# thucz/splatter360

Hardware: AMD Instinct MI355X
Metric: Msplats/s fwd+bwd @1M Gaussians, 1024x512 ERP (higher is better)
Workload: dtype f32; 1 GPU; BASELINE configs[2]: 1048576 encoder-like synthetic Gaussians (seed 0, deg-4 SH, from 2 context panoramas 1024x512), 1024x512 ERP = 6 faces 256x256 + stitch, fwdbwd, L2 loss on faces (fused epilogue, scalar reduced in the backward's first launch), lean tile lists; gaussians=1048576, face=256, views_per_gpu=1, parallelism=view-sharded x1, num_rendered=2237238, visible_pairs=1096454, split_lists=auto, split_quadrants=0, wide_rectangles=0, workspace_bytes_forward=1086440448, workspace_bytes_backward=1062934272, max_instances=2862083

## Files before the change

splatter360_amd/csrc/s360_forward.hip:

```cpp
#include "s360_device.h"
#include "s360_prof.h"
#include "s360_adapter_math.h"

#include <cstdio>
#include <cstdlib>

namespace s360 {

typedef float f4v __attribute__((ext_vector_type(4)));

template <bool CH_MAJOR, bool JAC>
__global__ __launch_bounds__(S360_BLOCK) void k_sh_eval(KParams kp, const S360View* __restrict__ views,
                                                       const float* __restrict__ means, const float* __restrict__ shs,
                                                       float4* __restrict__ rgbc, float* __restrict__ sh_jac,
                                                       uint32_t* __restrict__ zero_ptr, int zero_words) {
    const int g = blockIdx.x * S360_BLOCK + threadIdx.x;
    if (g < zero_words) zero_ptr[g] = 0u;
    if (g >= kp.P) return;
    const bool fast = kp.M == 25 && kp.deg == 4;
    const float* sh = shs + (size_t)g * kp.M * 3;
    float c[75];
    if (fast) load75(sh, c);
    const S360View& vw = views[0];
    const float sc = vw.scale;
// ... 682 lines not shown
        const uint32_t nch1 = nc1 > SORT_SHORT ? (nc1 + SORT_CHUNK - 1) / SORT_CHUNK : 0u;
        if (nch0 || nch1) atomicAdd(&lds_nlong, (nch0 ? 1u : 0u) + (nch1 ? 1u : 0u));
        uint32_t ctot;
        const uint32_t cex0 = block_exclusive_scan<TS_BLOCK / 64>(nch0 + nch1, lds, ctot), cex1 = cex0 + nch0;
        if (i0 < nt) {
            tile_start[i0] = carry + ex0;
            tile_cursor[i0] = 0;
            tile_max_contrib[i0] = 0;
            chunk_start[i0] = ccarry + cex0;
        }
        if (i1 < nt) {
            tile_start[i1] = carry + ex1;
            tile_cursor[i1] = 0;
            tile_max_contrib[i1] = 0;
            chunk_start[i1] = ccarry + cex1;
        }
        carry += tot;
        ccarry += ctot;
    }
    atomicMax(&lds_max, mx);
    __syncthreads();
    if (threadIdx.x == 0) {
        chunk_start[nt] = ccarry;
        tile_start[nt] = carry;
        header[0] = carry;
        header[1] = carry > cap ? 1u : 0u;
        header[2] = lds_max;
        {
            const uint32_t nmax = min(lds_max, cap);
            const uint32_t nch = nmax > SORT_SHORT ? (nmax + SORT_CHUNK - 1) / SORT_CHUNK : 0u;
            header[3] = merge_passes_of(nch);
        }
        header[4] = 0;
        *reinterpret_cast<SegBufs*>(header + S360_HDR_SEGBUFS) = sg_in;
        header[S360_HDR_SPLIT] = 0;
        header[6] = header[7] = 0;
        header[S360_HDR_SORT_ERR_TILE] = header[S360_HDR_SORT_ERR_PASS] = 0;
        if (header_mirror) __hip_atomic_store(header_mirror, (unsigned long long)carry | ((unsigned long long)(carry > cap ? 1u : 0u) << 32) |
                                                             ((unsigned long long)ccarry << 33),
                                              __ATOMIC_RELAXED, __HIP_MEMORY_SCOPE_SYSTEM);
        header[S360_HDR_NLONG] = lds_nlong;
        for (int i = 8; i < 25; ++i) header[i] = 0;
    }
}

#ifndef S360_EMIT_PPT
#define S360_EMIT_PPT 4
#endif
constexpr int EMIT_PPT = S360_EMIT_PPT;

template <bool LDS_BIN, bool COOP = false>
__global__ __launch_bounds__(S360_BLOCK) void k_emit(KParams kp, const uint32_t* __restrict__ tiles_touched,
                                                    const uint8_t* __restrict__ vis_mask, const float4* __restrict__ recA, const float4* __restrict__ recC,
                                                    const float* __restrict__ depths, const uint32_t* __restrict__ tile_start,
                                                    uint32_t* __restrict__ tile_cursor, uint64_t* __restrict__ keys,
                                                    uint2* __restrict__ slot_info, uint32_t* __restrict__ slot_pair,
                                                    uint32_t* __restrict__ slot_ticket, uint32_t* __restrict__ header,
                                                    uint32_t* __restrict__ long_pairs) {
    extern __shared__ __attribute__((aligned(16))) uint32_t lds_bin[];
    __shared__ uint32_t s_scan[S360_BLOCK / 64];
    __shared__ uint32_t s_slot0;
    const int v = blockIdx.y;
    const int g0 = blockIdx.x * (S360_BLOCK * EMIT_PPT) + threadIdx.x;
    const size_t tb = (size_t)image_of_view(kp, v) * kp.T;
    uint32_t* cnt = lds_bin;
    uint32_t* base = lds_bin + kp.T;
    const bool lean = (kp.flags & S360_FLAG_LEAN_LISTS) != 0;
    if (LDS_BIN) {
        for (int i = threadIdx.x; i < kp.T; i += S360_BLOCK) cnt[i] = 0u;
        __syncthreads();
    }
    __shared__ uint32_t s_p[S360_BLOCK * EMIT_PPT];
    uint32_t vis = 0;
#pragma unroll
    for (int j = 0; j < EMIT_PPT; ++j) {
        const int g = g0 + j * S360_BLOCK;
        if (g < kp.P && ((vis_mask[g] >> v) & 1u)) vis |= 1u << j;
    }
    uint32_t nvis;
    {
        uint32_t off = block_exclusive_scan((uint32_t)__builtin_popcount(vis), s_scan, nvis);
        for (uint32_t m = vis; m; m &= m - 1) s_p[off++] = (uint32_t)v * (uint32_t)kp.P + (uint32_t)(g0 + __builtin_ctz(m) * S360_BLOCK);
    }
    __syncthreads();
    uint32_t pr[EMIT_PPT], tt[EMIT_PPT], rlo[EMIT_PPT], rhi[EMIT_PPT], dbits[EMIT_PPT], hm[EMIT_PPT];
#pragma unroll
    for (int j = 0; j < EMIT_PPT; ++j) {
        const uint32_t e = threadIdx.x + j * S360_BLOCK;
        tt[j] = 0u; pr[j] = 0u; rlo[j] = rhi[j] = dbits[j] = 0u; hm[j] = 0xFFFFFFFFu;
        if (e < nvis) {
            const uint32_t p = s_p[e];
            const float4 rc = recA[3 * (size_t)p + 2];
            const float4 ra = recA[3 * (size_t)p];
            pr[j] = p;
            tt[j] = tiles_touched[p];
            dbits[j] = __float_as_uint(depths[p]);
            int minx, miny, maxx, maxy;
            tile_rect(ra.x, ra.y, __float_as_int(rc.y), kp.gx, kp.gy, minx, miny, maxx, maxy);
            rlo[j] = (uint32_t)minx | ((uint32_t)miny << 16);
            rhi[j] = (uint32_t)maxx | ((uint32_t)maxy << 16);
            if (lean && (maxx - minx) * (maxy - miny) <= 32) hm[j] = slot_info[p].y;
        }
    }
    uint32_t sl[EMIT_PPT], ticket = 0;
#pragma unroll
    for (int j = 0; j < EMIT_PPT; ++j) sl[j] = 0u;
    if (slot_pair) {
        uint32_t carry = 0;
#pragma unroll
        for (int j = 0; j < EMIT_PPT; ++j) {
            if ((uint32_t)j * S360_BLOCK >= nvis) break;
            uint32_t tot;
            sl[j] = carry + block_exclusive_scan(tt[j], s_scan, tot);
            carry += tot;
        }
        if (threadIdx.x == 0 && carry) ticket = tile_start[tb] + atomicAdd(&slot_ticket[image_of_view(kp, v) * 64], carry);
    }
    const int lane = threadIdx.x & 63;
    if (LDS_BIN) {
#pragma unroll
        for (int j = 0; j < EMIT_PPT; ++j) {
            if (COOP && (uint32_t)j * S360_BLOCK >= nvis) break;
            const bool wide = COOP && tt[j] > 32u;
            if (tt[j] && !wide) {
                const int minx = rlo[j] & 0xFFFFu, miny = rlo[j] >> 16, maxx = rhi[j] & 0xFFFFu, maxy = rhi[j] >> 16;
                uint32_t m = hm[j];
                for (int y = miny; y < maxy; ++y)
                    for (int x = minx; x < maxx; ++x) {
                        if (m & 1u) atomicAdd(&cnt[y * kp.gx + x], 1u);
                        m = (m >> 1) | 0x80000000u;
                    }
            }
            if (COOP) {
                for (unsigned long long big = __ballot(wide); big; big &= big - 1ull) {
                    const int src = (int)__builtin_ctzll(big);
                    const uint32_t lo = (uint32_t)__shfl((int)rlo[j], src), hi = (uint32_t)__shfl((int)rhi[j], src);
                    const int minx = lo & 0xFFFFu, miny = lo >> 16, w = (int)(hi & 0xFFFFu) - minx, n = w * ((int)(hi >> 16) - miny);
                    for (int i = lane; i < n; i += 64) {
                        const int y = i / w;
                        atomicAdd(&cnt[(miny + y) * kp.gx + minx + (i - y * w)], 1u);
                    }
                }
            }
        }
        __syncthreads();
        for (int i = threadIdx.x; i < kp.T; i += S360_BLOCK) {
            const uint32_t c = cnt[i];
            if (c) {
                base[i] = tile_start[tb + i] + atomicAdd(&tile_cursor[tb + i], c);
                cnt[i] = 0u;
            }
        }
    }
    if (slot_pair || LDS_BIN) {
        if (slot_pair && threadIdx.x == 0) s_slot0 = ticket;
        __syncthreads();
    }
#pragma unroll
    for (int j = 0; j < EMIT_PPT; ++j) {
        if (COOP && (uint32_t)j * S360_BLOCK >= nvis) break;
        const bool wide = COOP && tt[j] > 32u;
        const uint32_t p = pr[j];
        uint32_t slot = 0;
        if (tt[j]) {
            if (slot_pair) {
                slot = sl[j] + s_slot0;
                slot_info[p].x = slot;
            }
            if (tt[j] > 32u) {
                const uint32_t k = atomicAdd(&header[4], 1u);
                if (slot_pair && k < kp.cap / 32u + 1u) long_pairs[k] = p;
            }
        }
        const uint32_t ptag = p | (tt[j] > 32u ? 0x80000000u : 0u);
        if (tt[j] && !wide) {
            const int minx = rlo[j] & 0xFFFFu, miny = rlo[j] >> 16, maxx = rhi[j] & 0xFFFFu, maxy = rhi[j] >> 16;
            const uint64_t key = ((uint64_t)dbits[j] << 32) | (uint64_t)p;
            uint32_t m = hm[j];
            for (int y = miny; y < maxy; ++y)
                for (int x = minx; x < maxx; ++x) {
                    if (m & 1u) {
                        const int t = y * kp.gx + x;
                        const uint32_t pos = LDS_BIN ? base[t] + atomicAdd(&cnt[t], 1u)
                                                     : tile_start[tb + t] + atomicAdd(&tile_cursor[tb + t], 1u);
                        if (pos < kp.cap) keys[pos] = key;
                        if (slot_pair) {
                            if (slot < kp.cap) slot_pair[slot] = ptag;
                            ++slot;
                        }
                    }
                    m = (m >> 1) | 0x80000000u;
                }
        }
        if (COOP) {
            for (unsigned long long big = __ballot(wide); big; big &= big - 1ull) {
                const int src = (int)__builtin_ctzll(big);
                const uint32_t lo = (uint32_t)__shfl((int)rlo[j], src), hi = (uint32_t)__shfl((int)rhi[j], src);
                const uint32_t ps = (uint32_t)__shfl((int)p, src), ds = (uint32_t)__shfl((int)dbits[j], src), s0 = (uint32_t)__shfl((int)slot, src);
                const uint64_t key = ((uint64_t)ds << 32) | (uint64_t)ps;
                const int minx = lo & 0xFFFFu, miny = lo >> 16, w = (int)(hi & 0xFFFFu) - minx, n = w * ((int)(hi >> 16) - miny);
                for (int i = lane; i < n; i += 64) {
                    const int y = i / w;
                    const int t = (miny + y) * kp.gx + minx + (i - y * w);
                    const uint32_t pos = LDS_BIN ? base[t] + atomicAdd(&cnt[t], 1u)
                                                 : tile_start[tb + t] + atomicAdd(&tile_cursor[tb + t], 1u);
                    if (pos < kp.cap) keys[pos] = key;
                    if (slot_pair && s0 + (uint32_t)i < kp.cap) slot_pair[s0 + (uint32_t)i] = ps | 0x80000000u;
                }
            }
        }
    }
}

__device__ __forceinline__ uint64_t ld_dev(const uint64_t* p) { return __hip_atomic_load(p, __ATOMIC_RELAXED, __HIP_MEMORY_SCOPE_AGENT); }
__device__ __forceinline__ void st_dev(uint64_t* p, uint64_t v) { __hip_atomic_store(p, v, __ATOMIC_RELAXED, __HIP_MEMORY_SCOPE_AGENT); }

template <int THREADS, int E, bool DEV = false>
__device__ __forceinline__ void block_merge_sort(const uint64_t* __restrict__ in, uint64_t* __restrict__ out,
                                                 uint32_t* __restrict__ list, uint32_t n, uint64_t* lds_m) {
#define S360_PHYS(i) ((i) + (i) / E)
    const int tid = threadIdx.x;
    uint64_t k[E];
#pragma unroll
    for (int q = 0; q < E; ++q) {
        const uint32_t i = (uint32_t)(tid * E + q);
        k[q] = i < n ? in[i] : ~0ull;
    }
#pragma unroll
    for (int r = 0; r < E; ++r) {
#pragma unroll
        for (int q = (r & 1); q + 1 < E; q += 2) {
            const uint64_t a = k[q], b = k[q + 1];
            k[q] = a < b ? a : b;
            k[q + 1] = a < b ? b : a;
        }
    }
#pragma unroll
    for (int q = 0; q < E; ++q) lds_m[S360_PHYS((uint32_t)(tid * E + q))] = k[q];
#define S360_SORT_SYNC(w)                                                      \
    do {                                                                       \
        if (2u * (w) <= 64u * E) {                                             \
            __builtin_amdgcn_fence(__ATOMIC_RELEASE, "wavefront");             \
            __builtin_amdgcn_wave_barrier();                                   \
            __builtin_amdgcn_fence(__ATOMIC_ACQUIRE, "wavefront");             \
        } else {                                                               \
            __syncthreads();                                                   \
        }                                                                      \
    } while (0)
    S360_SORT_SYNC(E);
    uint32_t npad = E;
    while (npad < n) npad <<= 1;
    const uint32_t out0 = (uint32_t)tid * E;
    const bool live = out0 < n;
    for (uint32_t width = E; width < npad; width <<= 1) {
        const uint32_t pair = out0 / (2 * width) * (2 * width);
        const uint32_t pa = pair, pb = pair + width;
#define S360_A(x) lds_m[S360_PHYS(pa + (x))]
#define S360_B(x) lds_m[S360_PHYS(pb + (x))]
        if (live) {
            const uint32_t diag = out0 - pair;
            uint32_t lo_a = diag > width ? diag - width : 0u, hi_a = diag < width ? diag : width;
            while (lo_a < hi_a) {
                const uint32_t mid = (lo_a + hi_a) >> 1;
                if (S360_A(mid) <= S360_B(diag - 1 - mid)) lo_a = mid + 1; else hi_a = mid;
            }
            uint32_t a = lo_a, b = diag - lo_a;
            uint64_t ka = a < width ? S360_A(a) : ~0ull, kb = b < width ? S360_B(b) : ~0ull;
#pragma unroll
            for (int q = 0; q < E; ++q) {
                const bool take_a = ka <= kb;
                k[q] = take_a ? ka : kb;
                if (take_a) {
                    ++a;
                    ka = a < width ? S360_A(a) : ~0ull;
                } else {
                    ++b;
                    kb = b < width ? S360_B(b) : ~0ull;
                }
            }
        }
        S360_SORT_SYNC(width);
        if (live) {
#pragma unroll
            for (int q = 0; q < E; ++q) lds_m[S360_PHYS(out0 + q)] = k[q];
        }
        S360_SORT_SYNC(2u * width);
#undef S360_A
#undef S360_B
    }
    __syncthreads();
#undef S360_SORT_SYNC
#pragma unroll
    for (int q = 0; q < E; ++q) {
        const uint32_t i = (uint32_t)(tid * E + q);
        if (i < n) {
            const uint64_t kq = lds_m[S360_PHYS(i)];
            if (DEV) st_dev(out + i, kq); else out[i] = kq;
            if (list) list[i] = (uint32_t)kq;
        }
    }
#undef S360_PHYS
}


struct ChunkUnit {
    uint32_t s, n, k, passes, t;
    bool valid;
};
__device__ __forceinline__ ChunkUnit chunk_unit(const uint32_t* __restrict__ tile_start, const uint32_t* __restrict__ chunk_start,
                                                 int nt, uint32_t cap, uint32_t b) {
    ChunkUnit u;
    u.valid = b < chunk_start[nt];
    u.s = u.n = u.k = u.passes = u.t = 0;
    if (!u.valid) return u;
    const int lane = threadIdx.x & 63;
    int lo = 0, hi = nt;
    while (hi - lo > 1) {
        const int step = (hi - lo + 63) / 64;
        const int t = lo + lane * step;
        const bool p = t < hi && chunk_start[t] <= b;
        const int cnt = __popcll(__ballot(p));
        const int nhi = lo + cnt * step;
        lo = lo + (cnt - 1) * step;
        hi = nhi < hi ? nhi : hi;
    }
    u.s = min(tile_start[lo], cap);
    u.n = min(tile_start[lo + 1], cap) - u.s;
    u.k = b - chunk_start[lo];
    u.t = (uint32_t)lo;
    u.passes = merge_passes_of((u.n + SORT_CHUNK - 1) / SORT_CHUNK);
    return u;
}

__device__ __forceinline__ uint32_t merge_path_global_wave(const uint64_t* __restrict__ A, uint32_t la,
                                                           const uint64_t* __restrict__ B, uint32_t lb, uint32_t d, int lane) {
    uint32_t lo = d > lb ? d - lb : 0u, hi = d < la ? d : la;
    while (lo < hi) {
        const uint32_t step = (hi - lo + 63u) / 64u;
        const uint32_t a = lo + (uint32_t)lane * step;
        const bool p = a < hi && ld_dev(A + a) <= ld_dev(B + (d - 1 - a));
        const uint32_t cnt = (uint32_t)__popcll(__ballot(p));
        if (cnt == 0) {
            hi = lo;
        } else {
            const uint32_t nhi = lo + cnt * step;
            lo = lo + (cnt - 1) * step + 1;
            hi = nhi < hi ? nhi : hi;
        }
    }
    return lo;
}

__device__ __forceinline__ void merge_unit(const ChunkUnit& u, uint32_t pass, uint64_t* __restrict__ keys,
                                           uint64_t* __restrict__ alt, uint32_t* __restrict__ list, uint64_t* lds_m, uint32_t* s_part) {
    constexpr int THREADS = SORT_THREADS, E = 8;
#define S360_PHYS(i) ((i) + (i) / E)
    const uint32_t R = SORT_CHUNK << pass;
    const uint32_t o_tile = u.k * SORT_CHUNK, len = min(SORT_CHUNK, u.n - o_tile);
    const uint32_t pair0 = o_tile / (2 * R) * (2 * R);
    const uint32_t la = min(R, u.n - pair0), lb = min(R, u.n - pair0 - la);
    const uint64_t* src = (((u.passes - pass) & 1u) ? alt : keys) + u.s + pair0;
    uint64_t* dst = (((u.passes - pass - 1) & 1u) ? alt : keys) + u.s + o_tile;
    const uint64_t* A = src;
    const uint64_t* B = src + la;
    const uint32_t o = o_tile - pair0;
    if (threadIdx.x < 128) {
        const int w = threadIdx.x >> 6;
        const uint32_t r = merge_path_global_wave(A, la, B, lb, o + (uint32_t)w * len, threadIdx.x & 63);
        if ((threadIdx.x & 63) == 0) s_part[w] = r;
    }
    __syncthreads();
    const uint32_t a0 = s_part[0], a1 = s_part[1], b0 = o - a0, b1 = o + len - a1;
    const uint32_t na = a1 - a0, nb = b1 - b0;
    {
        uint64_t kin[E];
#pragma unroll
        for (int q = 0; q < E; ++q) {
            const uint32_t i = (uint32_t)threadIdx.x + (uint32_t)q * THREADS;
            kin[q] = i < len ? ld_dev(i < na ? A + (a0 + i) : B + (b0 + (i - na))) : 0ull;
        }
#pragma unroll
        for (int q = 0; q < E; ++q) {
            const uint32_t i = (uint32_t)threadIdx.x + (uint32_t)q * THREADS;
            if (i < len) lds_m[S360_PHYS(i)] = kin[q];
        }
    }
    __syncthreads();
    const uint32_t out0 = (uint32_t)threadIdx.x * E;
    if (out0 < len) {
        uint32_t lo_a = out0 > nb ? out0 - nb : 0u, hi_a = out0 < na ? out0 : na;
        while (lo_a < hi_a) {
            const uint32_t mid = (lo_a + hi_a) >> 1;
            if (lds_m[S360_PHYS(mid)] <= lds_m[S360_PHYS(na + out0 - 1 - mid)]) lo_a = mid + 1; else hi_a = mid;
        }
        uint32_t a = lo_a, b = out0 - lo_a;
        uint64_t ka = a < na ? lds_m[S360_PHYS(a)] : ~0ull, kb = b < nb ? lds_m[S360_PHYS(na + b)] : ~0ull;
        const bool last_pass = pass + 1 == u.passes;
        uint32_t* lst = list + u.s + o_tile;
#pragma unroll
        for (int q = 0; q < E; ++q) {
            const bool take_a = ka <= kb;
            const uint64_t kq = take_a ? ka : kb;
            if (take_a) {
                ++a;
                ka = a < na ? lds_m[S360_PHYS(a)] : ~0ull;
            } else {
                ++b;
                kb = b < nb ? lds_m[S360_PHYS(na + b)] : ~0ull;
            }
            if (out0 + q < len) {
                st_dev(dst + (out0 + q), kq);
                if (last_pass) lst[out0 + q] = (uint32_t)kq;
            }
        }
    }
#undef S360_PHYS
}

template <int THREADS>
__device__ __forceinline__ void sort_tiles_global_body(const uint32_t* __restrict__ tile_start, uint64_t* __restrict__ keys,
                                                       uint32_t* __restrict__ list, uint32_t lo, uint32_t cap, int nt,
                                                       uint32_t first, uint32_t stride) {
  for (int tile = (int)first; tile < nt; tile += (int)stride) {
    const uint32_t s = min(tile_start[tile], cap), e = min(tile_start[tile + 1], cap);
    const uint32_t n = e - s;
    if (n <= lo) continue;
    uint32_t npad = 1;
    while (npad < n) npad <<= 1;
    uint64_t* kk = keys + s;
    for (uint32_t k = 2; k <= npad; k <<= 1) {
        const uint32_t half = k >> 1;
        for (uint32_t t = threadIdx.x; t < (npad >> 1); t += THREADS) {
            const uint32_t blk = t / half, off = t - blk * half;
            const uint32_t i = blk * k + off, l = blk * k + (k - 1 - off);
            if (l < n) {
                const uint64_t a = kk[i], b = kk[l];
                if (a > b) {
                    kk[i] = b;
                    kk[l] = a;
                }
            }
        }
        __threadfence_block();
        __syncthreads();
        for (uint32_t j = k >> 2; j > 0; j >>= 1) {
            for (uint32_t t = threadIdx.x; t < (npad >> 1); t += THREADS) {
                const uint32_t i = ((t & ~(j - 1)) << 1) | (t & (j - 1)), l = i | j;
                if (l < n) {
                    const uint64_t a = kk[i], b = kk[l];
                    if (a > b) {
                        kk[i] = b;
                        kk[l] = a;
                    }
                }
            }
            __threadfence_block();
            __syncthreads();
        }
    }
    for (uint32_t i = threadIdx.x; i < n; i += THREADS) list[s + i] = (uint32_t)kk[i];
    __syncthreads();
  }
}

#ifndef S360_MERGE_BLOCKS
#define S360_MERGE_BLOCKS 256
#endif
__device__ __forceinline__ bool wait_count(const uint32_t* counter, uint32_t need) {
    uint32_t spins = 0;
    while (__hip_atomic_load(counter, __ATOMIC_RELAXED, __HIP_MEMORY_SCOPE_AGENT) < need) {
        if (++spins > (uint32_t)S360_SEGS_SPINS) return false;
        __builtin_amdgcn_s_sleep(32);
    }
    return true;
}
__device__ __forceinline__ void drain_stores_and_sync() {
    asm volatile("s_waitcnt vmcnt(0)" ::: "memory");
    __builtin_amdgcn_fence(__ATOMIC_RELEASE, "workgroup");
    __syncthreads();
}
__global__ __launch_bounds__(SORT_THREADS) void k_sort_stage1(const uint32_t* __restrict__ tile_start, const uint32_t* __restrict__ chunk_start,
                                                    int nt, uint64_t* __restrict__ keys, uint64_t* __restrict__ alt,
                                                    uint32_t* __restrict__ list, uint32_t cap, uint32_t max_passes, uint32_t cgrid,
                                                    const uint32_t* __restrict__ tile_count, uint32_t* __restrict__ tile_order,
                                                    uint32_t* __restrict__ header, unsigned long long* __restrict__ wide_mirror,
                                                    uint32_t* __restrict__ merge_done, uint32_t mgrid, uint32_t global_lo) {
    extern __shared__ __attribute__((aligned(16))) uint64_t lds_m[];
    uint32_t* const queue = merge_done + (size_t)nt * MAX_PASSES;
    uint32_t* const chunks_sorted = queue + 1;
    const uint32_t bid = blockIdx.x;
    if (bid < cgrid) {
        const uint32_t nchunks = chunk_start[nt];
        for (uint32_t b = bid; b < nchunks; b += cgrid) {
            const ChunkUnit u = chunk_unit(tile_start, chunk_start, nt, cap, b);
            if (u.valid && u.passes <= max_passes) {
                const uint32_t c0 = u.k * SORT_CHUNK, len = min(SORT_CHUNK, u.n - c0);
                uint64_t* dst = ((u.passes & 1u) ? alt : keys) + u.s + c0;
                if (u.passes == 0) {
                    block_merge_sort<SORT_THREADS, 8>(keys + u.s + c0, dst, list + u.s, len, lds_m);
                } else {
                    block_merge_sort<SORT_THREADS, 8, true>(keys + u.s + c0, dst, nullptr, len, lds_m);
                    drain_stores_and_sync();
                    if (threadIdx.x == 0) __hip_atomic_fetch_add(&chunks_sorted[u.t], 1u, __ATOMIC_RELAXED, __HIP_MEMORY_SCOPE_AGENT);
                }
            }
            __syncthreads();
        }
        return;
    }
    if (bid < cgrid + mgrid) {
        __shared__ uint32_t s_part[2];
        __shared__ uint32_t s_ticket;
        const uint32_t npass = min(header[3], max_passes);
        const uint32_t nchunks = npass ? chunk_start[nt] : 0u;
        const uint32_t nunits = npass * nchunks;
        while (bid - cgrid < nunits) {
            if (threadIdx.x == 0) s_ticket = __hip_atomic_fetch_add(queue, 1u, __ATOMIC_RELAXED, __HIP_MEMORY_SCOPE_AGENT);
            __syncthreads();
            const uint32_t tk = s_ticket;
            __syncthreads();
            if (tk >= nunits) break;
            const uint32_t pass = tk / nchunks, blk = tk - pass * nchunks;
            const ChunkUnit u = chunk_unit(tile_start, chunk_start, nt, cap, blk);
            if (!u.valid || u.passes > max_passes || pass >= u.passes) continue;
            const uint32_t nch = (u.n + SORT_CHUNK - 1) / SORT_CHUNK;
            if (threadIdx.x == 0) {
                const bool ok = wait_count(pass ? &merge_done[(size_t)u.t * MAX_PASSES + pass - 1] : &chunks_sorted[u.t], nch);
                if (!ok && atomicAdd(&header[7], 0x1000000u) < 0x1000000u) { header[S360_HDR_SORT_ERR_TILE] = u.t; header[S360_HDR_SORT_ERR_PASS] = pass; }
                s_ticket = ok ? 1u : 0u;
            }
            __syncthreads();
            const bool ok = s_ticket != 0u;
            __syncthreads();
            if (!ok) return;
            merge_unit(u, pass, keys, alt, list, lds_m, s_part);
            drain_stores_and_sync();
            if (threadIdx.x == 0 && pass + 1 < u.passes)
                __hip_atomic_fetch_add(&merge_done[(size_t)u.t * MAX_PASSES + pass], 1u, __ATOMIC_RELAXED, __HIP_MEMORY_SCOPE_AGENT);
        }
        if (header[2] > global_lo) sort_tiles_global_body<SORT_THREADS>(tile_start, keys, list, global_lo, cap, nt, bid - cgrid, mgrid);
        return;
    }
    if (bid < cgrid + mgrid + (uint32_t)nt) {
        const uint32_t tile = bid - cgrid - mgrid;
        const uint32_t s = min(tile_start[tile], cap), e = min(tile_start[tile + 1], cap);
        const uint32_t n = e - s;
        if (n == 0 || n > SORT_SHORT) return;
        block_merge_sort<SORT_THREADS, (int)(SORT_SHORT / SORT_THREADS)>(keys + s, keys + s, list + s, n, lds_m);
        return;
    }
    if (wide_mirror && threadIdx.x == 0) __hip_atomic_store(wide_mirror, (unsigned long long)header[4], __ATOMIC_RELAXED, __HIP_MEMORY_SCOPE_SYSTEM);
    if (tile_order) order_units_body<SORT_THREADS>(tile_count, tile_order, nt);
}

#ifndef S360_SPARSE_PIXELS
#define S360_SPARSE_PIXELS 6
#endif
constexpr int SPARSE_PIXELS = S360_SPARSE_PIXELS;

struct MseEp {
    const float* target;
    float* d_images;
    float* partials;
    float grad_scale;
    float* loss_out;
};

__global__ __launch_bounds__(MSE_BLOCK) void k_mse_finish(const float* __restrict__ partials, int n_per_view, int V, float loss_scale,
                                                         float inv_elems, float* __restrict__ out) {
    mse_finish_body(partials, n_per_view, V, loss_scale, inv_elems, out);
}


__device__ __forceinline__ void st_dev32(uint32_t* p, uint32_t v) { __hip_atomic_store(p, v, __ATOMIC_RELAXED, __HIP_MEMORY_SCOPE_AGENT); }
__device__ __forceinline__ uint32_t ld_dev32(const uint32_t* p) { return __hip_atomic_load(p, __ATOMIC_RELAXED, __HIP_MEMORY_SCOPE_AGENT); }
__device__ __forceinline__ void st_devf(float* p, float v) { st_dev32(reinterpret_cast<uint32_t*>(p), __float_as_uint(v)); }
__device__ __forceinline__ float ld_devf(const float* p) { return __uint_as_float(ld_dev32(reinterpret_cast<const uint32_t*>(p))); }

__device__ __forceinline__ void st_dev64(uint2* p, uint2 v) {
    __hip_atomic_store(reinterpret_cast<unsigned long long*>(p), (unsigned long long)v.x | ((unsigned long long)v.y << 32), __ATOMIC_RELAXED, __HIP_MEMORY_SCOPE_AGENT);
}
__device__ __forceinline__ uint2 ld_dev64(const uint2* p) {
    const unsigned long long v = __hip_atomic_load(reinterpret_cast<const unsigned long long*>(p), __ATOMIC_RELAXED, __HIP_MEMORY_SCOPE_AGENT);
    return make_uint2((uint32_t)v, (uint32_t)(v >> 32));
}
__device__ __forceinline__ float4 ld_dev_f4(const float4* p) {
    f4v r;
    asm volatile("global_load_dwordx4 %0, %1, off sc1\ns_waitcnt vmcnt(0)" : "=&v"(r) : "v"(p) : "memory");
    return make_float4(r.x, r.y, r.z, r.w);
}
__device__ __forceinline__ void st_dev_f4(float4* p, float4 v) {
    float* q = reinterpret_cast<float*>(p);
    st_devf(q, v.x); st_devf(q + 1, v.y); st_devf(q + 2, v.z); st_devf(q + 3, v.w);
}

struct WaveLds {
    float *x, *y, *a, *b, *c, *o;
    float2 *rg, *bz;
    uint32_t* pos;
};

template <bool WITH_DEPTH, bool T_ONLY>
__device__ __forceinline__ void composite_segment(const uint32_t* __restrict__ list, const float4* __restrict__ recA, const float* __restrict__ depths,
                                                  uint32_t start, uint32_t b0, uint32_t b1, float pxf, float pyf, float x0, float ys0, int lane,
                                                  const WaveLds& L, float inv_scale, float v_near, float v_far, int depth_mode, float& T, f2& C01,
                                                  f2& C2D, uint32_t& last, bool& done, float4* sv, uint32_t& scount) {
    uint32_t p_n1 = 0, p_n2 = 0;
    if (b0 + lane < b1) p_n1 = list[b0 + lane];
    if (b0 + 64 + lane < b1) p_n2 = list[b0 + 64 + lane];
    float4 na = make_float4(0.f, 0.f, 0.f, 0.f), nb = na, nc = na;
    float nz = 0.f;
    if (b0 + lane < b1) {
        na = recA[3 * (size_t)(p_n1)];
        nb = recA[3 * (size_t)(p_n1) + 1];
        nc = recA[3 * (size_t)(p_n1) + 2];
        if (WITH_DEPTH && !T_ONLY) nz = depths[p_n1];
    }
    for (uint32_t b = b0; b < b1; b += 64) {
        const unsigned long long act = __ballot(!done);
        if (act == 0ull) break;
        const float4 ea = na, eb = nb;
        float ez = 0.f;
        if (WITH_DEPTH && !T_ONLY) ez = depth_value(nz * inv_scale, v_near, v_far, depth_mode);
        const float ec = nc.x, erad = nc.y, eka = nc.z, ekb = nc.w;
        const bool ev = b + lane < b1;
        const uint32_t epair = p_n1;
        p_n1 = p_n2;
        if (b + 64 + lane < b1) {
            na = recA[3 * (size_t)(p_n1)];
            nb = recA[3 * (size_t)(p_n1) + 1];
            nc = recA[3 * (size_t)(p_n1) + 2];
            if (WITH_DEPTH && !T_ONLY) nz = depths[p_n1];
        }
        if (b + 128 + lane < b1) p_n2 = list[b + 128 + lane];
        const bool hit = ev && quadrant_hit(ea.x, ea.y, ea.z, ea.w, eb.x, eb.y, eka, ekb, x0, ys0);
        const unsigned long long m = __ballot(hit);
        if (m == 0ull) continue;
        const uint32_t rel = b - start;
        const uint32_t rank = __builtin_amdgcn_mbcnt_hi((uint32_t)(m >> 32), __builtin_amdgcn_mbcnt_lo((uint32_t)m, 0u));
        if (!T_ONLY && sv && hit) {
            float4* o = sv + 3 * (size_t)(scount + rank);
            o[0] = ea;
            o[1] = eb;
            o[2] = make_float4(ec, erad, __uint_as_float(rel + (uint32_t)lane), __uint_as_float(epair));
        }
        scount += (uint32_t)__popcll(m);
        if (__popcll(act) > SPARSE_PIXELS) {
            const uint32_t cnt = (uint32_t)__popcll(m);
            if (hit) {
                L.x[rank] = ea.x; L.y[rank] = ea.y; L.a[rank] = ea.z; L.b[rank] = ea.w;
                L.c[rank] = eb.x; L.o[rank] = eb.y;
                if (!T_ONLY) {
                    L.rg[rank] = make_float2(eb.z, eb.w);
                    L.bz[rank] = make_float2(ec, ez);
                    L.pos[rank] = rel + (uint32_t)lane + 1u;
                }
            }
            if (lane < 3) {
                L.x[cnt + lane] = 0.f; L.y[cnt + lane] = 0.f; L.a[cnt + lane] = 0.f; L.b[cnt + lane] = 0.f;
                L.c[cnt + lane] = 0.f; L.o[cnt + lane] = 0.f;
                if (!T_ONLY) {
                    L.rg[cnt + lane] = make_float2(0.f, 0.f);
                    L.bz[cnt + lane] = make_float2(0.f, 0.f);
                    L.pos[cnt + lane] = 0u;
                }
            }
            const f2 pxf2 = f2{pxf, pxf}, pyf2 = f2{pyf, pyf};
            for (uint32_t i = 0; i < cnt; i += 4) {
                const float4 vx = *reinterpret_cast<const float4*>(&L.x[i]), vy = *reinterpret_cast<const float4*>(&L.y[i]),
                             va = *reinterpret_cast<const float4*>(&L.a[i]), vb = *reinterpret_cast<const float4*>(&L.b[i]),
                             vc = *reinterpret_cast<const float4*>(&L.c[i]), vo = *reinterpret_cast<const float4*>(&L.o[i]);
                float al[4], om[4];
                bool ok[4];
                bool any_ok = false;
#pragma unroll
                for (int j = 0; j < 2; ++j) {
                    const f2 X = j ? f2{vx.z, vx.w} : f2{vx.x, vx.y}, Y = j ? f2{vy.z, vy.w} : f2{vy.x, vy.y};
                    const f2 A = j ? f2{va.z, va.w} : f2{va.x, va.y}, B = j ? f2{vb.z, vb.w} : f2{vb.x, vb.y};
                    const f2 Cc = j ? f2{vc.z, vc.w} : f2{vc.x, vc.y}, O = j ? f2{vo.z, vo.w} : f2{vo.x, vo.y};
                    const f2 dx = X - pxf2, dy = Y - pyf2;
                    const f2 t = pk_fma(B, dy, A * dx);
                    const f2 pw = pk_fma(t, dx, (Cc * dy) * dy);
                    const f2 og = O * f2{__builtin_amdgcn_exp2f(pw.x), __builtin_amdgcn_exp2f(pw.y)};
                    al[2 * j] = fminf(0.99f, og.x);
                    al[2 * j + 1] = fminf(0.99f, og.y);
                    const f2 o2 = f2{1.0f, 1.0f} - f2{al[2 * j], al[2 * j + 1]};
                    om[2 * j] = o2.x;
                    om[2 * j + 1] = o2.y;
                    ok[2 * j] = !done && !(pw.x > 0.0f) && !(al[2 * j] < 1.0f / 255.0f);
                    ok[2 * j + 1] = !done && !(pw.y > 0.0f) && !(al[2 * j + 1] < 1.0f / 255.0f);
                    any_ok = any_ok || ok[2 * j] || ok[2 * j + 1];
                }
                if (__ballot(any_ok) == 0ull) continue;
                if (T_ONLY) {
#pragma unroll
                    for (int e = 0; e < 4; ++e) {
                        const bool v = ok[e] && !done;
                        const float test_T = T * om[e];
                        const bool stop = v && test_T < 0.0001f;
                        done = done || stop;
                        T = (v && !stop) ? test_T : T;
                    }
                } else {
                    const float4 rg01 = *reinterpret_cast<const float4*>(&L.rg[i]), rg23 = *reinterpret_cast<const float4*>(&L.rg[i + 2]);
                    const float4 bz01 = *reinterpret_cast<const float4*>(&L.bz[i]), bz23 = *reinterpret_cast<const float4*>(&L.bz[i + 2]);
                    const uint4 vp = *reinterpret_cast<const uint4*>(&L.pos[i]);
                    const f2 rg[4] = {f2{rg01.x, rg01.y}, f2{rg01.z, rg01.w}, f2{rg23.x, rg23.y}, f2{rg23.z, rg23.w}};
                    const f2 bz[4] = {f2{bz01.x, bz01.y}, f2{bz01.z, bz01.w}, f2{bz23.x, bz23.y}, f2{bz23.z, bz23.w}};
                    const uint32_t posk[4] = {vp.x, vp.y, vp.z, vp.w};
#pragma unroll
                    for (int e = 0; e < 4; ++e) {
                        const bool v = ok[e] && !done;
                        const float test_T = T * om[e];
                        const bool stop = v && test_T < 0.0001f;
                        const bool contrib = v && !stop;
                        done = done || stop;
                        const float w = contrib ? al[e] * T : 0.0f;
                        const f2 w2 = f2{w, w};
                        C01 = C01 + rg[e] * w2;
                        if (WITH_DEPTH) C2D = C2D + bz[e] * w2;
                        else C2D.x = C2D.x + bz[e].x * w;
                        T = contrib ? test_T : T;
                        last = contrib ? posk[e] : last;
                    }
                }
            }
        } else {
            unsigned long long am = act;
            while (am) {
                const int pl = __builtin_ctzll(am);
                am &= am - 1;
                const float ppx = rl(pxf, pl), ppy = rl(pyf, pl);
                const float dx = ea.x - ppx, dy = ea.y - ppy;
                const float power = power2(ea.z, ea.w, eb.x, dx, dy);
                const float alpha = fminf(0.99f, eb.y * __builtin_amdgcn_exp2f(power));
                unsigned long long vm = __ballot(hit && !(power > 0.0f) && !(alpha < 1.0f / 255.0f));
                const bool mine = lane == pl;
                while (vm) {
                    const int eb_ = __builtin_ctzll(vm);
                    vm &= vm - 1;
                    const float a_s = rl(alpha, eb_);
                    const float test_T = T * (1.0f - a_s);
                    const bool stop = mine && test_T < 0.0001f;
                    const bool contrib = mine && !stop;
                    if (!T_ONLY) {
                        const float w = contrib ? a_s * T : 0.0f;
                        C01.x += rl(eb.z, eb_) * w;
                        C01.y += rl(eb.w, eb_) * w;
                        C2D.x += rl(ec, eb_) * w;
                        if (WITH_DEPTH) C2D.y += rl(ez, eb_) * w;
                        last = contrib ? rel + (uint32_t)eb_ + 1u : last;
                    }
                    T = contrib ? test_T : T;
                    done = done || stop;
                    if (__ballot(stop) != 0ull) break;
                }
            }
        }
    }
}

template <bool WITH_DEPTH, bool COH>
__device__ __forceinline__ void seg_item(const KParams& kp, const S360View* __restrict__ views, const uint32_t* __restrict__ tile_start,
                                         const uint32_t* __restrict__ list, const float4* __restrict__ recA, float* __restrict__ images,
                                         float* __restrict__ final_T, uint32_t* __restrict__ n_contrib, uint32_t* __restrict__ tile_max_contrib,
                                         uint32_t* __restrict__ strip_last, const float* __restrict__ depths, float* __restrict__ depth_maps,
                                         int depth_mode, const MseEp& ep, float4* __restrict__ surv, uint32_t* __restrict__ surv_count,
                                         const SegBufs& sg, int nt, uint32_t* __restrict__ dbg, const WaveLds& L, int lane, uint2 item, uint32_t wi,
                                         uint32_t nwork);

#ifndef S360_SPLIT_WAVES
#define S360_SPLIT_WAVES 4
#endif
#ifndef S360_P1_GRID
#define S360_P1_GRID 1024
#endif
#ifndef S360_P1_FIRST
#define S360_P1_FIRST 0
#endif
#ifndef S360_P2_GRID
#define S360_P2_GRID 1024
#endif
template <bool WITH_DEPTH, bool SPLIT>
__global__ __launch_bounds__(S360_BLOCK) __attribute__((amdgpu_waves_per_eu(SPLIT ? S360_SPLIT_WAVES : 6, SPLIT ? S360_SPLIT_WAVES : 6))) void k_render(KParams kp, const S360View* __restrict__ views,
                                                      const uint32_t* __restrict__ tile_start, const uint32_t* __restrict__ list,
                                                      const float4* __restrict__ recA, const float4* __restrict__ recB,
                                                      const float4* __restrict__ recC, float* __restrict__ images,
                                                      float* __restrict__ final_T, uint32_t* __restrict__ n_contrib,
                                                      uint32_t* __restrict__ tile_max_contrib, uint32_t* __restrict__ strip_last,
                                                      uint32_t* __restrict__ dbg, const float* __restrict__ depths,
                                                      float* __restrict__ depth_maps, int depth_mode, MseEp ep,
                                                      const uint32_t* __restrict__ tile_order, float4* __restrict__ surv,
                                                      uint32_t* __restrict__ surv_count, uint32_t* __restrict__ hdr_loss,
                                                      const SegBufs* __restrict__ sgp, const uint32_t* __restrict__ chunk_start,
                                                      unsigned long long* __restrict__ cand_mirror, int nt, const uint32_t* __restrict__ list_all,
                                                      const float* __restrict__ depths_all) {
#ifdef S360_DBG_TIMING
    const long long t_begin = wall_clock64();
#endif
    __shared__ __attribute__((aligned(16))) float s_x[S360_BLOCK / 64][68], s_y[S360_BLOCK / 64][68], s_a[S360_BLOCK / 64][68],
        s_b[S360_BLOCK / 64][68], s_c[S360_BLOCK / 64][68], s_o[S360_BLOCK / 64][68];
    __shared__ __attribute__((aligned(16))) float2 s_rg[S360_BLOCK / 64][68], s_bz[S360_BLOCK / 64][68];
    __shared__ __attribute__((aligned(16))) uint32_t s_pos[S360_BLOCK / 64][68];
    if (hdr_loss && blockIdx.x == 0 && threadIdx.x == 0) {
        const uint64_t pp = (uint64_t)(uintptr_t)ep.partials, po = (uint64_t)(uintptr_t)ep.loss_out;
        hdr_loss[0] = (uint32_t)pp; hdr_loss[1] = (uint32_t)(pp >> 32);
        hdr_loss[2] = (uint32_t)po; hdr_loss[3] = (uint32_t)(po >> 32);
        hdr_loss[4] = (uint32_t)(kp.T * 4); hdr_loss[5] = (uint32_t)kp.V;
        hdr_loss[6] = __float_as_uint(0.5f * ep.grad_scale);
        hdr_loss[7] = __float_as_uint(1.0f / (3.0f * (float)kp.H * (float)kp.W));
        for (int i = 0; i <= kp.V; ++i) ep.loss_out[i] = __uint_as_float(0x7FC00000u);
    }
    __shared__ uint32_t s_retired;
    uint32_t tile_slot = blockIdx.x;
    if (SPLIT) {
        const SegBufs& sgr = *sgp;
        const uint32_t n_long = S360_P1_FIRST ? sgr.header[S360_HDR_NLONG] : (uint32_t)nt;
        const uint32_t b = blockIdx.x;
        if (b >= n_long && b < n_long + (uint32_t)S360_P1_GRID) {
            const SegBufs sg = sgr;
            const int pwave = threadIdx.x >> 6, lane = threadIdx.x & 63;
            const WaveLds L{s_x[pwave], s_y[pwave], s_a[pwave], s_b[pwave], s_c[pwave], s_o[pwave], s_rg[pwave], s_bz[pwave], s_pos[pwave]};
            const uint32_t nunits = min((uint32_t)(SEG_PER_CHUNK * chunk_start[nt]), sg.n_slots);
            for (uint32_t u = b - n_long; u < nunits; u += (uint32_t)S360_P1_GRID) {
#ifdef S360_DBG_TIMING
                const long long t_p1 = wall_clock64();
#endif
                const ChunkUnit cu = chunk_unit(tile_start, chunk_start, nt, kp.cap, u / SEG_PER_CHUNK);
                const uint32_t k = cu.k * SEG_PER_CHUNK + (u % SEG_PER_CHUNK);
                if (!cu.valid || k < SEG_K0 || k * SEG_LEN >= cu.n || cu.n < SEG_HEAD + SEG_MIN_REST) continue;
                const int t1 = (int)cu.t, v1 = t1 / kp.T, rem1 = t1 - v1 * kp.T;
                const int ty1 = rem1 / kp.gx, tx1 = rem1 - ty1 * kp.gx;
                const int px1 = tx1 * 16 + sub_ox(pwave) + lane % SUB_W, py1 = ty1 * 16 + sub_oy(pwave) + lane / SUB_W;
                const bool inside1 = px1 < kp.W && py1 < kp.H;
                float T1 = 1.0f;
                f2 c01 = f2{0.f, 0.f}, c2d = f2{0.f, 0.f};
                uint32_t last1 = 0, cnt1 = 0;
                bool done1 = !inside1;
                const uint32_t b0 = cu.s + k * SEG_LEN, b1 = min(b0 + SEG_LEN, cu.s + cu.n);
                composite_segment<WITH_DEPTH, true>(list, recA, depths, cu.s, b0, b1, (float)px1, (float)py1, (float)(tx1 * 16 + sub_ox(pwave)),
                                                    (float)(ty1 * 16 + sub_oy(pwave)), lane, L, 0.f, 0.f, 0.f, depth_mode, T1, c01, c2d, last1, done1,
                                                    nullptr, cnt1);
                st_devf(sg.part_t + ((size_t)u * 4 + pwave) * 64 + lane, (done1 && inside1) ? 0.0f : T1);
                asm volatile("s_waitcnt vmcnt(0)" ::: "memory");
                if (lane == 0) __hip_atomic_fetch_add(&sg.seg_arrive[4 * t1 + pwave], 1u, __ATOMIC_RELAXED, __HIP_MEMORY_SCOPE_AGENT);
#ifdef S360_DBG_TIMING
                if (lane == 0) {
                    const size_t di = 4 * ((size_t)4 * nt + (size_t)4 * sg.n_slots + (size_t)u * 4 + pwave);
                    dbg[di] = (uint32_t)t_begin; dbg[di + 1] = (uint32_t)t_p1; dbg[di + 2] = (uint32_t)(wall_clock64() - t_p1);
                    dbg[di + 3] = ((uint32_t)t1 << 8) | k;
                }
// ... 937 lines not shown
```

Measured before the change: 1402 Msplats/s.

## Replace per-chunk block merge sort with LDS bucket sort plus merge fallback

Adds a block-level bucket sort that spreads keys across LDS buckets by their depth-key high word (min/max range scaled), ranks within small buckets by counting, and scatters them into place. It falls back to the existing merge sort when any bucket exceeds a small maximum. It is used for per-tile chunk sorts and for short-tile sorts, replacing the log-depth bitonic/merge network. The aim is fewer LDS passes and barriers, at the cost of an extra range reduction and data-dependent bucket skew.

```diff
diff --git a/splatter360_amd/csrc/s360_forward.hip b/splatter360_amd/csrc/s360_forward.hip
--- a/splatter360_amd/csrc/s360_forward.hip
+++ b/splatter360_amd/csrc/s360_forward.hip
@@ -1008,6 +1008,138 @@
 #undef S360_PHYS
 }
 
+#ifndef S360_SORT_BMAX
+#define S360_SORT_BMAX 16
+#endif
+constexpr size_t SORT_LDS_BYTES = (size_t)(8 * S360_SORT_THREADS + S360_SORT_THREADS) * 8;
+template <int THREADS, int E, int NB, bool DEV = false>
+__device__ __forceinline__ void block_bucket_sort(const uint64_t* __restrict__ in, uint64_t* __restrict__ out,
+                                                  uint32_t* __restrict__ list, uint32_t n, uint64_t* lds_m) {
+    constexpr int KEYS = THREADS * E, NW = THREADS / 64, C = NB / THREADS;
+    constexpr bool ALIAS = (size_t)KEYS * 8 + (size_t)NB * 4 + 256 > SORT_LDS_BYTES;
+    static_assert(NB % THREADS == 0 && (C == 4 || C == 8) && NW <= 16, "counters per thread: one or two 16-byte LDS accesses");
+    static_assert((size_t)KEYS * 8 + 256 <= SORT_LDS_BYTES && (size_t)NB * 4 <= (size_t)KEYS * 8, "LDS budget");
+    static_assert(KEYS <= 0x10000 && NB <= 0x10000 && KEYS <= 0x2000 && S360_SORT_BMAX < 0x80, "bucket | rank << 16; start | rank << 13 | count << 20");
+    uint64_t* const buf = lds_m;
+    uint32_t* const cnt = ALIAS ? (uint32_t*)lds_m : (uint32_t*)(lds_m + KEYS);
+    uint32_t* const red = ALIAS ? (uint32_t*)(lds_m + KEYS) : cnt + NB;
+    const int tid = threadIdx.x, lane = tid & 63, wave = tid >> 6;
+    uint64_t k[E];
+    uint32_t mn = ~0u, mx = 0u;
+#pragma unroll
+    for (int q = 0; q < E; ++q) {
+        const uint32_t i = (uint32_t)(tid + q * THREADS);
+        k[q] = in[min(i, n - 1u)];
+    }
+#pragma unroll
+    for (int j = 0; j < C / 4; ++j) ((uint4*)cnt)[tid * (C / 4) + j] = make_uint4(0u, 0u, 0u, 0u);
+#pragma unroll
+    for (int q = 0; q < E; ++q) {
+        const uint32_t h = (uint32_t)(k[q] >> 32);
+        mn = min(mn, h);
+        mx = max(mx, h);
+    }
+#pragma unroll
+    for (int off = 32; off > 0; off >>= 1) {
+        mn = min(mn, (uint32_t)__shfl_xor((int)mn, off));
+        mx = max(mx, (uint32_t)__shfl_xor((int)mx, off));
+    }
+    if (lane == 0) {
+        red[wave] = mn;
+        red[16 + wave] = mx;
+    }
+    __syncthreads();
+    uint32_t lo = ~0u, top = 0u;
+#pragma unroll
+    for (int w = 0; w < NW; ++w) {
+        lo = min(lo, red[w]);
+        top = max(top, red[16 + w]);
+    }
+    const float scale = (float)NB / ((float)(top - lo) + 1.0f);
+    uint32_t pk[E];
+#pragma unroll
+    for (int q = 0; q < E; ++q) {
+        const uint32_t i = (uint32_t)(tid + q * THREADS);
+        if (i < n) {
+            const uint32_t b = min((uint32_t)((float)((uint32_t)(k[q] >> 32) - lo) * scale), (uint32_t)(NB - 1));
+            pk[q] = b | (atomicAdd(&cnt[b], 1u) << 16);
+        }
+    }
+    __syncthreads();
+    uint32_t c[C], sum = 0u, big = 0u;
+#pragma unroll
+    for (int j = 0; j < C / 4; ++j) {
+        const uint4 v = ((const uint4*)cnt)[tid * (C / 4) + j];
+        c[4 * j] = v.x, c[4 * j + 1] = v.y, c[4 * j + 2] = v.z, c[4 * j + 3] = v.w;
+    }
+#pragma unroll
+    for (int j = 0; j < C; ++j) {
+        sum += c[j];
+        big = max(big, c[j]);
+    }
+    uint32_t incl = sum;
+#pragma unroll
+    for (int off = 1; off < 64; off <<= 1) {
+        const uint32_t up = (uint32_t)__shfl_up((int)incl, off);
+        if (lane >= off) incl += up;
+    }
+    if (lane == 63) red[32 + wave] = incl;
+    if (__syncthreads_or(big > (uint32_t)S360_SORT_BMAX)) {
+        block_merge_sort<THREADS, E, DEV>(in, out, list, n, lds_m);
+        return;
+    }
+    uint32_t run = incl - sum;
+#pragma unroll
+    for (int w = 0; w < NW; ++w) run += w < wave ? red[32 + w] : 0u;
+#pragma unroll
+    for (int j = 0; j < C; ++j) {
+        const uint32_t cj = c[j];
+        c[j] = run | (cj << 20);
+        run += cj;
+    }
+#pragma unroll
+    for (int j = 0; j < C / 4; ++j) ((uint4*)cnt)[tid * (C / 4) + j] = make_uint4(c[4 * j], c[4 * j + 1], c[4 * j + 2], c[4 * j + 3]);
+    __syncthreads();
+#pragma unroll
+    for (int q = 0; q < E; ++q) {
+        const uint32_t i = (uint32_t)(tid + q * THREADS);
+        if (i < n) pk[q] = cnt[pk[q] & 0xFFFFu] | (pk[q] >> 16 << 13);
+    }
+    if (ALIAS) __syncthreads();
+#pragma unroll
+    for (int q = 0; q < E; ++q) {
+        const uint32_t i = (uint32_t)(tid + q * THREADS);
+        if (i < n) buf[(pk[q] & 0x1FFFu) + ((pk[q] >> 13) & 0x7Fu)] = k[q];
+    }
+    __syncthreads();
+#pragma unroll
+    for (int q = 0; q < E; ++q) {
+        const uint32_t i = (uint32_t)(tid + q * THREADS);
+        if (i < n) {
+            const uint32_t s = pk[q] & 0x1FFFu, e = s + (pk[q] >> 20);
+            uint32_t below = 0u;
+            for (uint32_t j = s; j < e; ++j) below += buf[j] < k[q] ? 1u : 0u;
+            pk[q] = s + below;
+        }
+    }
+    __syncthreads();
+#pragma unroll
+    for (int q = 0; q < E; ++q) {
+        const uint32_t i = (uint32_t)(tid + q * THREADS);
+        if (i < n) buf[pk[q]] = k[q];
+    }
+    __syncthreads();
+#pragma unroll
+    for (int q = 0; q < E; ++q) {
+        const uint32_t i = (uint32_t)(tid + q * THREADS);
+        if (i < n) {
+            const uint64_t kq = buf[i];
+            if (DEV) st_dev(out + i, kq); else out[i] = kq;
+            if (list) list[i] = (uint32_t)kq;
+        }
+    }
+}
+
 
 struct ChunkUnit {
     uint32_t s, n, k, passes, t;
@@ -1185,6 +1317,18 @@
     __builtin_amdgcn_fence(__ATOMIC_RELEASE, "workgroup");
     __syncthreads();
 }
+#ifndef S360_SORT_BUCKET_CHUNKS
+#define S360_SORT_BUCKET_CHUNKS 1
+#endif
+template <bool DEV>
+__device__ __forceinline__ void sort_chunk(const uint64_t* __restrict__ in, uint64_t* __restrict__ out, uint32_t* __restrict__ list,
+                                           uint32_t n, uint64_t* lds_m) {
+#if S360_SORT_BUCKET_CHUNKS
+    block_bucket_sort<SORT_THREADS, 8, (int)SORT_CHUNK, DEV>(in, out, list, n, lds_m);
+#else
+    block_merge_sort<SORT_THREADS, 8, DEV>(in, out, list, n, lds_m);
+#endif
+}
 __global__ __launch_bounds__(SORT_THREADS) void k_sort_stage1(const uint32_t* __restrict__ tile_start, const uint32_t* __restrict__ chunk_start,
                                                     int nt, uint64_t* __restrict__ keys, uint64_t* __restrict__ alt,
                                                     uint32_t* __restrict__ list, uint32_t cap, uint32_t max_passes, uint32_t cgrid,
@@ -1203,9 +1347,9 @@
                 const uint32_t c0 = u.k * SORT_CHUNK, len = min(SORT_CHUNK, u.n - c0);
                 uint64_t* dst = ((u.passes & 1u) ? alt : keys) + u.s + c0;
                 if (u.passes == 0) {
-                    block_merge_sort<SORT_THREADS, 8>(keys + u.s + c0, dst, list + u.s, len, lds_m);
+                    sort_chunk<false>(keys + u.s + c0, dst, list + u.s, len, lds_m);
                 } else {
-                    block_merge_sort<SORT_THREADS, 8, true>(keys + u.s + c0, dst, nullptr, len, lds_m);
+                    sort_chunk<true>(keys + u.s + c0, dst, nullptr, len, lds_m);
                     drain_stores_and_sync();
                     if (threadIdx.x == 0) __hip_atomic_fetch_add(&chunks_sorted[u.t], 1u, __ATOMIC_RELAXED, __HIP_MEMORY_SCOPE_AGENT);
                 }
@@ -1252,7 +1396,7 @@
         const uint32_t s = min(tile_start[tile], cap), e = min(tile_start[tile + 1], cap);
         const uint32_t n = e - s;
         if (n == 0 || n > SORT_SHORT) return;
-        block_merge_sort<SORT_THREADS, (int)(SORT_SHORT / SORT_THREADS)>(keys + s, keys + s, list + s, n, lds_m);
+        block_bucket_sort<SORT_THREADS, (int)(SORT_SHORT / SORT_THREADS), (int)SORT_SHORT>(keys + s, keys + s, list + s, n, lds_m);
         return;
     }
     if (wide_mirror && threadIdx.x == 0) __hip_atomic_store(wide_mirror, (unsigned long long)header[4], __ATOMIC_RELAXED, __HIP_MEMORY_SCOPE_SYSTEM);
```

Result: faster. 1440 Msplats/s (median of 6 runs) (+2.7%).
